# jianhengLiu/VINS-RGBD-FAST

Measured on AMD Instinct MI355X. Metric: VIO frames/sec (640x480, 150 feats, 10-KF window), higher is better.
Workload: dtype f64; 1 GPU; BASELINE configs[2]: 128 independent synthetic 640x480 RGB-D + 200 Hz IMU sequences per MI355X, 150 features, 10-keyframe window; sequences_per_gpu=128, tracker_lag=1, parallelism=sequences sharded per GPU, no data-path collective

## Files before the change

### vins-rgbd-fast_amd/csrc/be_linalg.h

```cpp
#pragma once
#include <hip/hip_runtime.h>
#include "vio_state.h"

namespace {

__device__ __forceinline__ double dpp_f64(double v, const int ctrl_tag) {
    int lo = __double2loint(v), hi = __double2hiint(v);
    switch (ctrl_tag) {
    case 0: lo = __builtin_amdgcn_update_dpp(0, lo, 0xB1, 0xF, 0xF, true); hi = __builtin_amdgcn_update_dpp(0, hi, 0xB1, 0xF, 0xF, true); break;
    case 1: lo = __builtin_amdgcn_update_dpp(0, lo, 0x4E, 0xF, 0xF, true); hi = __builtin_amdgcn_update_dpp(0, hi, 0x4E, 0xF, 0xF, true); break;
    case 2: lo = __builtin_amdgcn_update_dpp(0, lo, 0x141, 0xF, 0xF, true); hi = __builtin_amdgcn_update_dpp(0, hi, 0x141, 0xF, 0xF, true); break;
    default: lo = __builtin_amdgcn_update_dpp(0, lo, 0x140, 0xF, 0xF, true); hi = __builtin_amdgcn_update_dpp(0, hi, 0x140, 0xF, 0xF, true); break;
    }
    return __hiloint2double(hi, lo);
}
__device__ __forceinline__ double rl_f64(double v, int src_lane) {
    int lo = __double2loint(v), hi = __double2hiint(v);
    lo = __builtin_amdgcn_readlane(lo, src_lane);
    hi = __builtin_amdgcn_readlane(hi, src_lane);
    return __hiloint2double(hi, lo);
}
__device__ __forceinline__ double wave_sum_dpp(double v) {
    v += dpp_f64(v, 0);
    v += dpp_f64(v, 1);
// ... 1411 lines not shown
            WAVE_SYNC();
            if (lane < 16) xs[16 * p + lane] = x;
        }
        __syncthreads();
        for (int q = t; q < 16 * p; q += nt) {
            int tj = q >> 4, cc = q & 15;
            double sacc = 0;
#pragma unroll
            for (int k = 0; k < 16; k++) sacc += T[tl_idx(p, tj, k, cc)] * xs[16 * p + k];
            xs[q] -= sacc;
        }
        __syncthreads();
    }
}

__device__ __forceinline__ void chol_backward_tiles_wave(const double *T, int nb, double *xs, const double *dinv) {
    const int lane = threadIdx.x & 63, wave = threadIdx.x >> 6;
    if (wave == 0) {
        const int c = lane & 15;
        for (int p = nb - 1; p >= 0; p--) {
            const double *D = T + ((size_t)(p * (p + 1) / 2 + p) << 8);
            double m[16], b[16];
#pragma unroll
            for (int k = 0; k < 16; k++) { m[k] = D[(c << 4) + (k ^ c)]; b[k] = xs[16 * p + k]; }
            const double dv = dinv[16 * p + c];
            double x = 0;
#pragma unroll
            for (int k = 0; k < 16; k++) x += (k > c ? m[k] : (k == c ? dv : 0.0)) * b[k];
            WAVE_SYNC();
            if (lane < 16) xs[16 * p + lane] = x;
            WAVE_SYNC();
#pragma unroll
            for (int k = 0; k < 16; k++) b[k] = xs[16 * p + k];
            for (int q = lane; q < 16 * p; q += 64) {
                const int tj = q >> 4, cc = q & 15;
#pragma unroll
                for (int k = 0; k < 16; k++) m[k] = T[tl_idx(p, tj, k, cc)];
                double sacc = 0;
#pragma unroll
                for (int k = 0; k < 16; k++) sacc += m[k] * b[k];
                xs[q] -= sacc;
            }
            WAVE_SYNC();
        }
    }
    __syncthreads();
}

__device__ __forceinline__ void chol_solve_tiles(const double *T, int nb, double *xs, const double *dinv) {
    const int t = threadIdx.x, nt = blockDim.x, lane = t & 63, wave = t >> 6;
    for (int p = 0; p < nb; p++) {
        if (wave == 0) {
            const int row = lane & 15;
            double b = xs[16 * p + row];
#pragma unroll
            for (int j = 0; j < 16; j++) {
                double xj = bcast_lane(b, j) * dinv[16 * p + j];
                if (row == j) b = xj; else if (row > j) b -= T[tl_idx(p, p, row, j)] * xj;
            }
            if (lane < 16) xs[16 * p + row] = b;
// ... 293 lines not shown
        for (int a = t; a < n; a += nt) {
            double sacc = 0;
            if (a < n0 || (a >= e0 && a < e0 + ne))
                for (int q = 0; q < nw; q++) sacc += part[q * VIO_LWMAX + a];
            out_col[a] = sacc;
        }
    }
    __syncthreads();
}
template <int RB = 4>
__device__ __forceinline__ void matvec_pass_2range(const double *M, int ld, int nrows, int n, int n0, int e0, int ne, const double *u, const double *v,
                                                   double *out_col, double *out_row, double *part) {
    if (n0 + ne <= 128) matvec_pass_2range_t<2, RB>(M, ld, nrows, n, n0, e0, ne, u, v, out_col, out_row, part);
    else matvec_pass_t<6>(M, ld, nrows, n, u, v, out_col, out_row, part);
}
template <int RB = 4>
__device__ __forceinline__ void matvec_pass(const double *M, int ld, int nrows, int n, const double *u, const double *v, double *out_col, double *out_row,
                            double *part) {
    if (n <= 192) matvec_pass_t<3, RB>(M, ld, nrows, n, u, v, out_col, out_row, part);
    else matvec_pass_t<6>(M, ld, nrows, n, u, v, out_col, out_row, part);
}

}
```

### vins-rgbd-fast_amd/csrc/be_phased.h

```cpp
#define PS_LDS_TILE_DOUBLES 16896

namespace {

#define PS_LS_HEAD_DOUBLES (((int)(sizeof(Params) / sizeof(double)) + 1 & ~1) + 176)
#define PS_LVEC 14
__device__ __forceinline__ bool ps_active(const SolveSt &st) { return st.stage != PS_IDLE && st.stage != PS_DONE; }
__device__ __forceinline__ double *ps_imu_blk(const Ctx &c) { return c.pairblk + (size_t)((c.W + 1) * c.W / 2) * 210; }
__device__ __forceinline__ unsigned ps_colmask(int W1, int LW, bool vext) {
    unsigned m = 0;
    for (int cb = 0; cb < (LW >> 4); cb++) {
        const int c0 = 16 * cb, c1 = c0 + 15;
        if (c0 < 6 * W1 || (vext && c1 >= 15 * W1 && c0 < 15 * W1 + 7)) m |= 1u << cb;
    }
    return m;
}

__device__ __forceinline__ int fis_early(const SolveSt &st, int chunk, int pslot) { return st.fi[chunk][pslot]; }
__device__ __forceinline__ void ps_sel_rows(const Batch &B, Ctx &c, int buf) {
    if (!buf) return;
    const size_t S = (size_t)B.S, n8 = (size_t)c.NL + 8;
    c.Hpl += S * n8 * c.LW; c.Hll += S * n8; c.gl += S * n8;
}

}
// ... 143 lines not shown
            st.cost = ccost;
            st.succ++;
            if (rel < 0.25) st.radius *= 0.5;
            if (rel > 0.75) st.radius = fmax(st.radius, 3.0 * st.dogleg_norm);
            st.mu = fmax(1e-8, 2.0 * st.mu / 10.0);
            st.point_new = 1;
            if (st.fused && st.eval_with_J) st.rowbuf ^= 1;
            st.stage = st.iter >= cfg.max_iterations ? PS_DONE : PS_ASM;
        } else {
            st.radius *= 0.5;
            st.stage = st.iter >= cfg.max_iterations ? PS_DONE : PS_STEP;
        }
    }
}

__device__ __forceinline__ void ps_form_candidate(const Ctx &c, SolveSt &st, const double alpha, const double *delta, const double *stl, const double *sl, double *sred) {
    const int t = threadIdx.x, nt = blockDim.x;
    const vio_config &cfg = c.C->c;
    const int W = c.W, W1 = W + 1, oE = 15 * W1, oT = 15 * W1 + 6;
    const int F = st.F, Fa = st.Fa, ex_active = st.ex_active, td_active = st.td_active;
    const int *alist = c.pair_list + c.nres_cap - c.NL;
    const Params &X = st.X;
    Params &Xc = st.Xc;
    double xn2 = 0, dn2 = 0, ncl = 0;
    if (t <= W) {
        double pc[7], d6[6];
        for (int k = 0; k < 7; k++) pc[k] = X.pose[t * 7 + k];
        for (int k = 0; k < 6; k++) d6[k] = alpha * delta[6 * t + k];
        bf::pose_plus(pc, d6);
        for (int k = 0; k < 7; k++) { const double v = X.pose[t * 7 + k], d = v - pc[k]; xn2 += v * v; dn2 += d * d; Xc.pose[t * 7 + k] = pc[k]; }
        for (int k = 0; k < 9; k++) {
// ... 2 lines not shown
            Xc.sb[t * 9 + k] = vc;
        }
    }
    if (t == W + 1) {
        const bool relo = st.relo != 0;
        double ec[7], d6[6];
        for (int k = 0; k < 7; k++) ec[k] = relo ? X.relo[k] : X.ex[k];
        for (int k = 0; k < 6; k++) d6[k] = alpha * delta[oE + k];
        if (ex_active) bf::pose_plus(ec, d6);
        const double tdc = X.td + (td_active ? alpha * delta[oT] : 0.0);
        if (ex_active) for (int k = 0; k < 7; k++) { const double v = relo ? X.relo[k] : X.ex[k], d = v - ec[k]; xn2 += v * v; dn2 += d * d; }
        if (td_active) { xn2 += X.td * X.td; dn2 += (X.td - tdc) * (X.td - tdc); }
        for (int k = 0; k < 7; k++) { Xc.ex[k] = relo ? X.ex[k] : ec[k]; Xc.relo[k] = relo ? ec[k] : X.relo[k]; }
        Xc.td = tdc;
    }
    for (int k = t; k < F; k += nt) c.cfeat[k] = c.feat[k];
    __syncthreads();
    for (int k = t; k < Fa; k += nt) {
        int slot = alist[k], pi = c.lm_pidx[slot];
        const double v0 = c.feat[pi];
        double v = v0 + alpha * (stl[k] * sl[k]);
        double ub = (c.lm_est[slot] == 2) ? 2.0 / cfg.depth_max : 1.7976931348623157e308;
        if (v > ub) { v = ub; ncl += 1; }
        c.cfeat[pi] = v;
        xn2 += v0 * v0; dn2 += (v0 - v) * (v0 - v);
    }
    block_sum3(xn2, dn2, ncl, sred);
    if (t == 0) { st.step_xn2 = xn2; st.step_dn2 = dn2; if (ncl > 0) c.be->bound_clamps += (int)ncl; }
}

__device__ __forceinline__ bool ps_blk(const Batch &B, int &s, int &b) {
    if (B.xcd_nb == 0) { s = (int)blockIdx.y + B.s0; b = (int)blockIdx.x; return true; }
    const int L = (int)blockIdx.x, X = B.xcd_n, idx = L / X, sl = idx / B.xcd_nb, r = sl * X + (L - idx * X);
    b = idx - sl * B.xcd_nb;
    s = r + B.s0;
    return r < B.ns;
}
// ... 1292 lines not shown
    double *out = c.vec + 7 * LW;
    const int n0 = 6 * W1, e0 = 15 * W1, ne = st.vext ? 7 : 0;
    if (n0 + ne <= 128) ps_colsum_as_eight_waves<2, 8>(c.Hpl, LW, Fa, P, n0, e0, ne, wk_s, out, part);
    else ps_colsum_as_eight_waves<3, 8>(c.Hpl, LW, Fa, P, n0, e0, ne, wk_s, out, part);
}

__global__ __launch_bounds__(256, 5) void ps_asm_b_schur_kernel(Batch B, int nb_b, int by_blocks) {
    int s, b;
    if (!ps_blk(B, s, b)) return;
    extern __shared__ double ps_wk_s[];
    if (B.gn_ext && b == nb_b + B.n_schur) ps_gn_rhs_body(B, s, ps_wk_s);
    else if (b < nb_b) { if (by_blocks == 1) ps_asm_b_blocks(B, s, b, nb_b); else if (by_blocks == 2) ps_asm_b_body(B, s, b, nb_b, true); else ps_asm_b_body(B, s, b, nb_b, false); }
    else ps_schur_body(B, s, b - nb_b, ps_wk_s);
}

template <bool BIG, int TB> __device__ __forceinline__ void ps_serial_body(const Batch &B) {
    const int s = blockIdx.x + B.s0, t = threadIdx.x, nt = blockDim.x;
    SolveSt &st = B.sst[s];
    if (st.stage != PS_ASM && st.stage != PS_SCHUR && st.stage != PS_STEP) return;
    Ctx c = make_ctx(B, s);
    ps_sel_rows(B, c, st.rowbuf);
    const vio_config &cfg = c.C->c;
    const int W = c.W, W1 = W + 1, P = c.P, LW = c.LW;
    __shared__ double sred[64];
    __shared__ int sh_i[8];
    __shared__ double chol_dinv[VIO_LWMAX];
    extern __shared__ __attribute__((aligned(16))) unsigned char smem[];
    double *xs = (double *)smem, *work = xs + LW;
    const int F = st.F, Fa = st.Fa;
    const int ex_active = st.ex_active, td_active = st.td_active;
    const int ne_ext = st.vext ? 7 : 0;
// ... 7 lines not shown
           *yp = lv + 11 * LW, *up = lv + 12 * LW, *tmpv2 = lv + 13 * LW;
    double *sl = c.lvec, *dgl = c.lvec + c.NLs, *gradl = c.lvec + 2 * c.NLs, *gnl = c.lvec + 3 * c.NLs, *stl = c.lvec + 4 * c.NLs,
           *inv = c.lvec + 5 * c.NLs, *gls = c.lvec + 6 * c.NLs, *Hlls = c.lvec + 7 * c.NLs;
    const int Kpad = (Fa + 3) & ~3;
    double *hsgl = c.res + (size_t)c.nres_cap * 42 - 4 * (size_t)c.NLs;
    double *yl = hsgl + c.NLs, *ul = yl + c.NLs, *tmpl = ul + c.NLs;
    const int stage0 = st.stage;
    const bool s_formed = B.form_s && stage0 == PS_ASM && st.scale_pending == 0;
    double radius = st.radius, mu = st.mu, alpha = st.alpha, dogleg_norm = st.dogleg_norm;
    bool cauchy_valid = st.cauchy_valid != 0;
    int invalid = st.invalid;
    int iter = st.iter;
    if (!st.retry) iter++;
    PH_INIT;
    const bool have_lv = !(iter > cfg.max_iterations);
    if (have_lv) for (int i = t; i < PS_LVEC * LW; i += nt) lv[i] = c.vec[i];
    __syncthreads();
    auto finish = [&](int new_stage) {
        __syncthreads();
        if (have_lv) for (int i = 2 * LW + t; i < PS_LVEC * LW; i += nt) c.vec[i] = lv[i];
        if (t == 0) {
            st.radius = radius; st.mu = mu; st.alpha = alpha; st.dogleg_norm = dogleg_norm; st.cauchy_valid = cauchy_valid ? 1 : 0;
            st.invalid = invalid; st.iter = iter; st.stage = new_stage;
        }
    };
    if (iter > cfg.max_iterations) { if (t == 0) st.iters_done = cfg.max_iterations; iter = cfg.max_iterations; finish(PS_DONE); return; }
    if (t == 0) { st.iters_done = iter; st.retry = 0; }
    if (stage0 == PS_ASM || stage0 == PS_SCHUR) {
        if (st.scale_pending) {
            for (int k = t; k < Kpad; k += nt) sl[k] = k < Fa ? 1.0 / (1.0 + sqrt(c.Hll[k])) : 0.0;
            __syncthreads();
            if (t == 0) st.scale_pending = 0;
        }
        if (st.point_new) {
            double m = 0;
            for (int a = t; a < P; a += nt) m = fmax(m, sp[a] != 0.0 ? fabs(g[a]) : 0.0);
            for (int k = t; k < Fa; k += nt) m = fmax(m, fabs(c.gl[k]));
            const double gmax = block_max(m, sred);
            for (int a = t; a < LW; a += nt) {
                double hs = a < P ? sp[a] * sp[a] * c.H[a * LW + a] : 0.0;
                gs[a] = a < P ? sp[a] * g[a] : 0.0;
                dgp[a] = sqrt(fmin(fmax(hs, 1e-6), 1e32));
                gradp[a] = gs[a] / dgp[a];
                sgp[a] = gradp[a] / dgp[a];
                up[a] = sp[a] * sgp[a];
            }
            for (int k = t; k < Kpad; k += nt) {
                double hl = k < Fa ? sl[k] * sl[k] * c.Hll[k] : 0.0;
                Hlls[k] = hl;
                gls[k] = k < Fa ? sl[k] * c.gl[k] : 0.0;
                dgl[k] = sqrt(fmin(fmax(hl, 1e-6), 1e32));
                gradl[k] = gls[k] / dgl[k];
                ul[k] = sl[k] * (gradl[k] / dgl[k]);
            }
            __syncthreads();
            if (t == 0) st.point_new = 0;
            if (gmax <= 1e-10) { if (t == 0) st.iters_done = iter - 1; finish(PS_DONE); return; }
        }
        PH(48);
        cauchy_valid = false;
        for (int k = t; k < Kpad; k += nt) {
            double iv = k < Fa ? 1.0 / (Hlls[k] + mu * dgl[k] * dgl[k]) : 0.0;
            inv[k] = iv;
            if (!B.gn_ext) tmpl[k] = sl[k] * iv * gls[k];
        }
        __syncthreads();
        if (!B.gn_ext) matvec_pass_2range<TB>(c.Hpl, LW, Fa, P, 6 * W1, 15 * W1, ne_ext, tmpl, nullptr, tmpv, nullptr, work);
        for (int a = t; a < LW; a += nt) xs[a] = a < P ? gs[a] - sp[a] * tmpv[a] : 0.0;
        __syncthreads();
        PH(49);
        constexpr bool big = BIG;
        double *Stiles = big ? c.Sc : work;
        if (s_formed) {
            if (!big) {
                const int nd2 = (LW >> 4) * ((LW >> 4) + 1) / 2 * 128;
                const double2 *src = (const double2 *)c.Sc;
                double2 *dst = (double2 *)work;
                for (int i0 = t; i0 < nd2; i0 += 8 * nt) {
                    double2 v[8];
#pragma unroll
                    for (int u = 0; u < 8; u++) v[u] = src[min(i0 + u * nt, nd2 - 1)];
#pragma unroll
                    for (int u = 0; u < 8; u++) if (i0 + u * nt < nd2) dst[i0 + u * nt] = v[u];
                }
                __syncthreads();
            }
        } else {
            const unsigned colmask = ps_colmask(W1, LW, st.vext != 0);
            const int nb = LW >> 4, ntile = nb * (nb + 1) / 2;
// ... 18 lines not shown
                    sr[b] = sp[row]; sc0[b] = sp[col]; sc1[b] = sp[col + 1]; dg[b] = dgp[row];
                }
#pragma unroll
                for (int b = 0; b < TB; b++) {
                    if (tile0 + b * tstep >= ntile) break;
                    const double u0 = swp ? uv[b].y : uv[b].x, u1 = swp ? uv[b].x : uv[b].y;
                    double v0 = sr[b] * sc0[b] * (hv[b].x - u0), v1 = sr[b] * sc1[b] * (hv[b].y - u1);
                    if (dia0[b]) { v0 += mu * dg[b] * dg[b]; if (sr[b] == 0.0) v0 = 1.0; }
                    if (dia1[b]) { v1 += mu * dg[b] * dg[b]; if (sr[b] == 0.0) v1 = 1.0; }
                    *(double2 *)&Stiles[widx[b]] = swp ? make_double2(v1, v0) : make_double2(v0, v1);
                }
            }
            __syncthreads();
        }
        PH(50);
        bool ok = big ? chol_tiles_stream(c.Sc, LW >> 4, work, &sh_i[2], chol_dinv, xs)
                      : chol_tiles(work, LW >> 4, &sh_i[2], chol_dinv, s == 0 ? B.timings + 59 : nullptr, xs);
        PH(51);
        if (st.test_fail > 0) { ok = false; __syncthreads(); if (t == 0) st.test_fail--; }
        if (ok) {
            chol_backward_tiles_wave(big ? c.Sc : work, LW >> 4, xs, chol_dinv);
            PH(56);
            double bad = 0;
            for (int a = t; a < P; a += nt) if (!isfinite(xs[a])) bad += 1;
            bad = block_sum(bad, sred);
            ok = bad == 0;
        }
        if (!ok) {
            mu *= 10.0;
            if (mu < 1.0) { if (t == 0) st.retry = 1; finish(PS_SCHUR); return; }
            finish(PS_DONE);
            return;
        }
        PH(57);
        for (int a = t; a < LW; a += nt) { yp[a] = xs[a]; gnp[a] = -xs[a] * dgp[a]; tmpv[a] = sp[a] * xs[a]; }
        __syncthreads();
        matvec_pass_2range<TB>(c.Hpl, LW, Fa, P, 6 * W1, 15 * W1, ne_ext, nullptr, tmpv, nullptr, tmpl, nullptr);
        PH(58);
        for (int k = t; k < Kpad; k += nt) {
            double y = k < Fa ? (gls[k] - sl[k] * tmpl[k]) * inv[k] : 0.0;
            yl[k] = y;
            gnl[k] = -y * dgl[k];
        }
        __syncthreads();
    }
    PH(52);
    double gnorm = 0, gnn = 0, gdot = 0;
    for (int a = t; a < P; a += nt) { gnorm += gradp[a] * gradp[a]; gnn += gnp[a] * gnp[a]; gdot += gradp[a] * gnp[a]; }
    for (int k = t; k < Fa; k += nt) { gnorm += gradl[k] * gradl[k]; gnn += gnl[k] * gnl[k]; gdot += gradl[k] * gnl[k]; }
    block_sum3(gnorm, gnn, gdot, sred);
    gnorm = sqrt(gnorm);
    gnn = sqrt(gnn);
// ... 52 lines not shown
        }
    }
    block_sum3(n2, lin, quad, sred);
    if (dogleg_norm < 0) dogleg_norm = sqrt(n2);
    const double model_change = -(lin + 0.5 * quad);
    if (!(model_change > 0)) {
        if (++invalid >= 5) { finish(PS_DONE); return; }
        mu *= 10.0;
        finish(PS_SCHUR);
        return;
    }
    invalid = 0;
    PH(54);
    for (int a = t; a < LW; a += nt) delta[a] = a < P ? stp[a] * sp[a] : 0.0;
    __syncthreads();
    ps_form_candidate(c, st, 1.0, delta, stl, sl, sred);
    if (t == 0) st.ls_pending = st.constrained;
    if (t == 0) { st.model_change = model_change; st.eval_with_J = iter < cfg.max_iterations ? 1 : 0; }
    finish(PS_EVAL_C);
    PH(55);
}

__global__ __launch_bounds__(512) void ps_serial_kernel_512(Batch B) { ps_serial_body<false, 8>(B); }
__global__ __launch_bounds__(512) void ps_serial_big_kernel(Batch B) { ps_serial_body<true, 8>(B); }

__global__ __launch_bounds__(256, 2) void ps_ls_kernel(Batch B) {
    const int s = blockIdx.x + B.s0, t = threadIdx.x, nt = blockDim.x;
    SolveSt &st = B.sst[s];
    if (st.stage != PS_EVAL_C || !st.ls_pending) return;
    extern __shared__ __attribute__((aligned(16))) unsigned char lds[];
    __shared__ double sred[64];
    Ctx c = make_ctx(B, s);
    ps_sel_rows(B, c, st.rowbuf);
    const BeSeq &be = *c.be;
    const vio_config &cfg = c.C->c;
    const int W = c.W, W1 = W + 1, P = c.P, Fa = st.Fa, nblk = min(PS_MAX_EVAL_BLOCKS, 3 + (st.nres + 256 * B.eval_rpt - 1) / (256 * B.eval_rpt));
    constexpr int XD = ((int)(sizeof(Params) / sizeof(double)) + 1) & ~1;
    Params &X = *(Params *)lds;
    double *lsw = (double *)lds + XD, *lpart = lsw + 104;
// ... 90 lines not shown
```

### vins-rgbd-fast_amd/csrc/kernels.h

```cpp
#pragma once
#include <hip/hip_runtime.h>
#include "vio_state.h"
#include "../../include/vio_synth.h"

#define PI_CH 8
#define PREINT_MANY_LDS_DOUBLES (PI_CH * (225 + 270))
static inline size_t fast_lds_bytes(int rw, int rh) {
    return (size_t)(((rw + 6) * rh + 15) & ~15) + (size_t)((rw * rh + 15) & ~15) + (size_t)(((rw - 6) * (rh - 6) + 63) / 64 + 2) * 8 + 16;
}
__host__ __device__ static inline size_t ps_eval_lds_bytes(int W) {
    const size_t W1 = (size_t)W + 1, a = (W1 * W1 + 1) * 32 * 8, b = (size_t)W * (VIO_PREINT_HDR + 1) * 8;
    return (a > b ? a : b) + 64;
}
static inline size_t ps_ls_lds_bytes(int W) { (void)W; return ((((sizeof(Params) / sizeof(double)) + 1) & ~(size_t)1) + 176) * 8 + 16; }
struct LkImages {
    const uint8_t *prev[4];
    const uint8_t *next[4];
    int w[4], h[4];
};

__global__ void fe_begin_kernel(Batch B, const double *stamps, int gate, int publish, const uint8_t *modes, const double *R_rel);
__global__ void be_latest_odometry_kernel(Batch B, int seq, double *out11);
__global__ void fe_predict_motion_kernel(Batch B, int seq, double t0, double t1, double *out9);
__global__ void fe_pyrdown_kernel(Batch B, const uint8_t *src_base, size_t src_stride, int sw, int sh, int dst_level, int write_level0);
// ... 21 lines not shown
template <bool EXCALIB> __global__ void be_ingest_kernel(Batch B, const uint16_t *depth_base, size_t depth_stride, IngestSrc src);
__global__ void be_stage_relative_r_kernel(int n, const double *corres6, double *R9);
__global__ void be_solve_kernel(Batch B);
__global__ void be_solve_kernel_512(Batch B);
__global__ void be_marg_kernel(Batch B);
__global__ void be_marg_exact_kernel(Batch B);
__global__ void ps_setup_kernel(Batch B);
__global__ void ps_eval_kernel(Batch B);
__global__ void ps_eval_kernel_occ3(Batch B);
__global__ void ps_eval_kernel_occ4(Batch B);
__global__ void ps_asm_a_kernel(Batch B);
__global__ void ps_asm_a_kernel_occ4(Batch B);
__global__ void ps_asm_b_schur_kernel(Batch B, int nb_b, int by_blocks);
__global__ void ps_serial_big_kernel(Batch B);
__global__ void ps_serial_kernel_512(Batch B);
__global__ void ps_final_kernel(Batch B);
__global__ void ps_ls_kernel(Batch B);
__global__ void ps_evalf_kernel(Batch B);
static inline size_t ps_evalf_lds_bytes(int W) {
    const size_t W1 = (size_t)W + 1, a = ((size_t)PS_FUSE_CAP * 28 + (W1 * W / 2 + 1) * 32) * 8 + (size_t)PS_FUSE_CAP * 12, b = ((size_t)W * (VIO_PREINT_HDR + 1) + (size_t)W * 465) * 8;
    return (a > b ? a : b) + 16;
}
__global__ void be_prior_factor_kernel(Batch B, int seq);
__global__ void be_set_relo_kernel(Batch B, int seq, const double *par);
__global__ void be_stage_pnp_kernel(const double *pts, int n, double *par6);
__global__ void be_dyn_finalize_kernel(Batch B, int seq, const double *samples, const int *offs);
__global__ void be_stage_imu_kernel(vio_config cfg, PreInt *P, int n, const double *dt, const double *acc, const double *gyr,
                                    const double *par, double g_norm, double *preint_out, double *r15, double *J480);
__global__ void be_stage_projection_kernel(vio_config cfg, const double *in, int use_td, int form, double *r2, double *J46);
__global__ void be_stage_imu_block_kernel(const PreInt *P, const double *par, double g_norm, double *G961);
// ... 4 lines not shown
```

### vins-rgbd-fast_amd/csrc/vio_abi.hip

```cpp
#include <hip/hip_runtime.h>
#include <math.h>
#include <algorithm>
#include <cmath>
#include <stdlib.h>
#include <mutex>
#include <chrono>
#include <string>
#include <string.h>
#include <vector>
#include "kernels.h"
#include "dyninit_host.h"
#include "camera_model.h"
#include "snapshot.h"

thread_local std::string g_err;

namespace {

#define HIPCHK(x)                                                                                        \
    do {                                                                                                 \
        hipError_t e_ = (x);                                                                             \
        if (e_ != hipSuccess) { g_err = std::string(#x) + ": " + hipGetErrorString(e_); return VIO_EDEVICE; } \
    } while (0)

// ... 97 lines not shown
        bool busy = false;
    } imu_stage[2];
    int imu_stage_cur = 0;
    hipEvent_t ev_imu = nullptr;
    std::vector<double> last_imu_t;
    size_t lds_select = 0, lds_add = 0, lds_fast = 0, lds_solve = 0, lds_serial = 0, lds_marg = 0, lds_factor = 0, lds_ps_ls = 0, lds_ps_evalf = 0;
    int ps_evalf_blocks = 0;
    bool feed_throttle = true;
    int uploads_in_flight = 2;
    int relo_frames = 0;
    bool line_search = true;
    int be_threads = 512, marg_threads = 384;
    int solve_mode = 1;
    bool asm_a_occ4 = false;
    int eval_occ = 0;
    bool serial_big = false;
    size_t lds_ps_eval = 0;
    int ps_eval_blocks = 0, ps_asm_a_blocks = 0, ps_schur_tiles = 0;
    bool timing_valid = false;
    std::vector<hipEvent_t> pev;
    int prof_steps = 0, prof_cur = -1;
    bool prof_fe_only = false;
    struct SnapRow { const char *name; int kind; unsigned char *base; int64_t bytes, blob_off; };
    std::vector<SnapRow> snap_rows;
    int64_t snap_dev_bytes = 0, snap_chunks = 0;
    int snap_entries = 0;
    SnapEntry *d_snap_tab = nullptr;
    SnapSeq *d_snap_seqs = nullptr;
    size_t snap_seqs_cap = 0;
    unsigned char *d_snap_stage = nullptr;
// ... 516 lines not shown
            const dim3 g_e = xm ? dim3(S8 * nb_e) : dim3(nb_e, S), g_a = xm ? dim3(S8 * nb_a) : dim3(nb_a, S), g_b = xm ? dim3(S8 * nb_bs) : dim3(nb_bs, S);
            Batch Bf = Bg;
            Bf.ns = S; Bf.xcd_n = XN; Bf.xcd_nb = xm ? h->ps_evalf_blocks : 0;
            const dim3 g_f = xm ? dim3(S8 * h->ps_evalf_blocks) : dim3(h->ps_evalf_blocks, S);
            for (int k = 0; k < slots; k++) {
                if (Bg.fuse) ps_evalf_kernel<<<g_f, 256, h->lds_ps_evalf, st>>>(Bf);
                if (!fuse_only) {
                    if (h->eval_occ == 4) ps_eval_kernel_occ4<<<g_e, 256, h->lds_ps_eval, st>>>(Be);
                    else if (h->eval_occ == 3) ps_eval_kernel_occ3<<<g_e, 256, h->lds_ps_eval, st>>>(Be);
                    else ps_eval_kernel<<<g_e, 256, h->lds_ps_eval, st>>>(Be);
                    if (h->asm_a_occ4) ps_asm_a_kernel_occ4<<<g_a, 512, 0, st>>>(Ba);
                    else ps_asm_a_kernel<<<g_a, 512, 0, st>>>(Ba);
                }
                ps_asm_b_schur_kernel<<<g_b, 256, (size_t)(C.NL + 16 + (6 * (C.W + 1) + 7 <= 128 ? 8 * 128 : 8 * 192) ) * sizeof(double), st>>>(Bb, h->ps_asm_b_blocks, h->asm_b_by_blocks);
                if (h->serial_big) ps_serial_big_kernel<<<S, 512, h->lds_serial, st>>>(Bg);
                else ps_serial_kernel_512<<<S, 512, h->lds_serial, st>>>(Bg);
                if (h->line_search && k + 1 < slots) ps_ls_kernel<<<S, 256, h->lds_ps_ls, st>>>(Bg);
            }
            ps_final_kernel<<<S, 256, 0, st>>>(Bg);
        };
        if (h->use_graph && one_seq < 0) {
            uint64_t key = 1469598103934665603ULL;
            auto mixin = [&](const void *p, size_t nbytes) { const unsigned char *q = (const unsigned char *)p; for (size_t i = 0; i < nbytes; i++) { key ^= q[i]; key *= 1099511628211ULL; } };
            mixin(&Bg, sizeof(Bg));
            mixin(&h->line_search, sizeof(h->line_search));
            mixin(&fuse_only, sizeof(fuse_only));
            const int knobs[12] = {C.c.max_iterations + h->extra_slots, h->eval_occ, h->asm_a_occ4 ? 1 : 0, h->serial_big ? 1 : 0, h->serial_threads, h->ps_eval_blocks, h->ps_asm_a_blocks,
                                   h->ps_asm_b_blocks + 1000 * h->asm_b_by_blocks, h->ps_schur_tiles, h->xcd_map, h->xcd_n, (int)h->lds_serial};
            mixin(knobs, sizeof(knobs));
            mixin(&h->lds_ps_eval, sizeof(h->lds_ps_eval));
            if (g.solve_graph && g.solve_graph_key != key) { (void)hipGraphExecDestroy(g.solve_graph); g.solve_graph = nullptr; }
            g.solve_graph_key = key;
            if (!g.solve_graph) {
                hipGraph_t gr = nullptr;
                HIPCHK(hipStreamBeginCapture(st, hipStreamCaptureModeThreadLocal));
                launch_phased();
                HIPCHK(hipStreamEndCapture(st, &gr));
                HIPCHK(hipGraphInstantiate(&g.solve_graph, gr, nullptr, nullptr, 0));
                (void)hipGraphDestroy(gr);
            }
            HIPCHK(hipGraphLaunch(g.solve_graph, st));
        } else
// ... 316 lines not shown
            if (C.NPRIOR <= 96) workd = std::max(workd, (size_t)C.NPRIOR * (C.NPRIOR | 1) + 2);
            {
                size_t nb = (size_t)C.LW >> 4, tiles = nb * (nb + 1) / 2 * 256;
                if (tiles <= 16896) workd = std::max(workd, tiles);
            }
            h->lds_solve = ((size_t)C.LW + 2 + workd) * 8 + 16;
            (void)raise_lds_limit((const void *)be_solve_kernel, (size_t)(h->lds_solve));
            (void)raise_lds_limit((const void *)be_solve_kernel_512, (size_t)(h->lds_solve));
            {
                const size_t nb = (size_t)C.LW >> 4, tiles = nb * (nb + 1) / 2 * 256;
                const size_t wk = std::max(tiles <= 16896 ? tiles : (2 * nb + 1) * 256, (size_t)16 * 336);
                h->serial_big = tiles > 16896;
                h->B.form_s = (getenv("VIO_FORM_S") ? atoi(getenv("VIO_FORM_S")) != 0 : true) && h->asm_b_by_blocks == 2;
                h->lds_serial = ((size_t)C.LW + 2 + wk + 2 + (size_t)14  * C.LW) * 8 + 16;
                if (getenv("VIO_SERIAL_LDS") && (size_t)atol(getenv("VIO_SERIAL_LDS")) > h->lds_serial) h->lds_serial = (size_t)atol(getenv("VIO_SERIAL_LDS"));
                (void)raise_lds_limit(h->serial_big ? (const void *)ps_serial_big_kernel : (const void *)ps_serial_kernel_512, h->lds_serial);
            }
            {
                const size_t nb = (size_t)C.LW >> 4, tiles = nb * (nb + 1) / 2 * 256, W1 = (size_t)C.W + 1;
                const bool eligible = !(B.flags & 1) && (size_t)C.W * C.NP / 256 + 4 <= PS_MAX_EVAL_BLOCKS &&
                                      (size_t)C.W * 768 <= (W1 * W1 - W1 * C.W / 2) * 210 && nb <= 32;
                h->solve_mode = getenv("VIO_SOLVE_MODE") ? atoi(getenv("VIO_SOLVE_MODE")) : 1;
                if (!eligible) h->solve_mode = 0;
                h->lds_ps_eval = ps_eval_lds_bytes(C.W);
                (void)raise_lds_limit((const void *)ps_eval_kernel, h->lds_ps_eval);
                h->lds_ps_evalf = ps_evalf_lds_bytes(C.W);
                {
                    const int want = getenv("VIO_FUSE") ? atoi(getenv("VIO_FUSE")) : 0;
                    int chunks = (int)std::min<size_t>(PS_FUSE_MAXBLK, (W1 * (size_t)C.c.max_cnt * 11 / 10 + (PS_FUSE_CAP - C.W) - 1) / (PS_FUSE_CAP - C.W));
                    if (want > 1) chunks = std::min(PS_FUSE_MAXBLK, want);
                    B.fuse = (want && C.W <= PS_FUSE_MAXW && C.c.use_imu && B.pairpart) ? std::max(1, chunks) : 0;
// ... 29 lines not shown
        (void)raise_lds_limit((const void *)be_marg_kernel, (size_t)(h->lds_marg));
        (void)raise_lds_limit((const void *)be_marg_exact_kernel, (size_t)(h->lds_marg));
        const bool excalib = C.c.estimate_extrinsic == 2;
        const void *ingest = excalib ? (const void *)be_ingest_kernel<true> : (const void *)be_ingest_kernel<false>;
        (void)raise_lds_limit(ingest, ingest_lds_bytes(C, excalib));

        (void)raise_lds_limit((const void *)fe_select_kernel, (size_t)(h->lds_select));
        (void)raise_lds_limit((const void *)fe_add_kernel, (size_t)(h->lds_add));
        (void)raise_lds_limit((const void *)fe_fast_kernel, (size_t)(h->lds_fast));
        bool fits = lds_fits(C.MX > 0 ? (const void *)be_marg_exact_kernel : (const void *)be_marg_kernel, h->lds_marg, "be_marg") &&
                    lds_fits(ingest, ingest_lds_bytes(C, excalib), "be_ingest") &&
                    lds_fits((const void *)fe_select_kernel, h->lds_select, "fe_select") && lds_fits((const void *)fe_add_kernel, h->lds_add, "fe_add") &&
                    lds_fits((const void *)fe_fast_kernel, h->lds_fast, "fe_fast");
        if (fits && h->solve_mode == 1)
            fits = lds_fits((const void *)ps_eval_kernel, h->lds_ps_eval, "ps_eval") && lds_fits((const void *)ps_ls_kernel, h->lds_ps_ls, "ps_ls") &&
                   lds_fits(h->serial_big ? (const void *)ps_serial_big_kernel : (const void *)ps_serial_kernel_512, h->lds_serial, "ps_serial");
        else if (fits)
            fits = lds_fits(h->be_threads <= 512 ? (const void *)be_solve_kernel_512 : (const void *)be_solve_kernel, h->lds_solve, "be_solve");
        if (!fits) rc = VIO_ECAPACITY;
    }
    if (rc != VIO_OK) { vio_destroy(h); return nullptr; }
    return h;
}

void vio_destroy(vio_batch *h) {
    if (!h) return;
    int caller_dev = -1;
    const bool dev_switched = h->device >= 0 && hipGetDevice(&caller_dev) == hipSuccess && caller_dev != h->device && hipSetDevice(h->device) == hipSuccess;
    (void)hipDeviceSynchronize();
    for (void *p : h->allocs) (void)hipFree(p);
    if (h->d_gray_stage) (void)hipFree(h->d_gray_stage);
// ... 1658 lines not shown
```

Before: 60270 frames/s.

## Overlap serial-solve loads with compute via async LDS DMA and register prefetch

Adds an overlapped variant of the phased serial solver kernel, on by default and switchable with VIO_SERIAL_OVERLAP. At kernel start it issues global_load_lds DMA of the Schur tiles into LDS and prefetches per-thread scalars (Hll, gl, H diagonal, feature values, landmark indices) into registers so later stages skip those global reads. During the single-wave Cholesky back-substitution, the other waves prefetch Hpl rows into registers for the following row-dot pass. This hides global memory latency behind serial work, at the cost of higher register pressure in a 512-thread kernel and extra code complexity.

```diff
diff --git a/vins-rgbd-fast_amd/csrc/be_linalg.h b/vins-rgbd-fast_amd/csrc/be_linalg.h
--- a/vins-rgbd-fast_amd/csrc/be_linalg.h
+++ b/vins-rgbd-fast_amd/csrc/be_linalg.h
@@ -1449,9 +1449,9 @@
     }
 }
 
-__device__ __forceinline__ void chol_backward_tiles_wave(const double *T, int nb, double *xs, const double *dinv) {
-    const int lane = threadIdx.x & 63, wave = threadIdx.x >> 6;
-    if (wave == 0) {
+__device__ __forceinline__ void chol_backward_tiles_wave0(const double *T, int nb, double *xs, const double *dinv) {
+    const int lane = threadIdx.x & 63;
+    {
         const int c = lane & 15;
         for (int p = nb - 1; p >= 0; p--) {
             const double *D = T + ((size_t)(p * (p + 1) / 2 + p) << 8);
@@ -1479,6 +1479,9 @@
             WAVE_SYNC();
         }
     }
+}
+__device__ __forceinline__ void chol_backward_tiles_wave(const double *T, int nb, double *xs, const double *dinv) {
+    if ((threadIdx.x >> 6) == 0) chol_backward_tiles_wave0(T, nb, xs, dinv);
     __syncthreads();
 }
 
@@ -1802,6 +1805,64 @@
     if (n0 + ne <= 128) matvec_pass_2range_t<2, RB>(M, ld, nrows, n, n0, e0, ne, u, v, out_col, out_row, part);
     else matvec_pass_t<6>(M, ld, nrows, n, u, v, out_col, out_row, part);
 }
+template <int PR>
+__device__ __forceinline__ void rowdot_2range_prefetch(const double *M, int ld, int nrows, int n0, int e0, int ne, double (&m)[PR][2]) {
+    const int lane = threadIdx.x & 63, wave = threadIdx.x >> 6, nw = blockDim.x >> 6;
+    const int ncomp = n0 + ne;
+    int col[2];
+#pragma unroll
+    for (int j = 0; j < 2; j++) { const int q = lane + 64 * j; col[j] = q < n0 ? q : (q < ncomp ? e0 + (q - n0) : -1); }
+#pragma unroll
+    for (int b = 0; b < PR; b++) {
+        const double *r = M + (size_t)max(min((wave - 1) + (nw - 1) * b, nrows - 1), 0) * ld;
+#pragma unroll
+        for (int j = 0; j < 2; j++) m[b][j] = col[j] >= 0 ? r[col[j]] : 0.0;
+    }
+}
+template <int PR, int RB>
+__device__ __forceinline__ void rowdot_2range_finish(const double *M, int ld, int nrows, int n0, int e0, int ne, const double *v, double *out_row, const double (&m)[PR][2]) {
+    const int lane = threadIdx.x & 63, wave = threadIdx.x >> 6, nw = blockDim.x >> 6;
+    const int ncomp = n0 + ne;
+    int col[2];
+    double vv[2];
+#pragma unroll
+    for (int j = 0; j < 2; j++) {
+        const int q = lane + 64 * j;
+        col[j] = q < n0 ? q : (q < ncomp ? e0 + (q - n0) : -1);
+        vv[j] = col[j] >= 0 ? v[col[j]] : 0.0;
+    }
+    if (wave > 0) {
+#pragma unroll
+        for (int b = 0; b < PR; b++) {
+            const int k = (wave - 1) + (nw - 1) * b;
+            double rd = 0;
+#pragma unroll
+            for (int j = 0; j < 2; j++) rd += m[b][j] * vv[j];
+            rd = wave_sum_dpp(rd);
+            if (lane == 0 && k < nrows) out_row[k] = rd;
+        }
+    }
+    for (int k0 = (nw - 1) * PR + wave; k0 < nrows; k0 += RB * nw) {
+        double mr[RB][2];
+#pragma unroll
+        for (int b = 0; b < RB; b++) {
+            const double *r = M + (size_t)min(k0 + b * nw, nrows - 1) * ld;
+#pragma unroll
+            for (int j = 0; j < 2; j++) mr[b][j] = col[j] >= 0 ? r[col[j]] : 0.0;
+        }
+#pragma unroll
+        for (int b = 0; b < RB; b++) {
+            const int k = k0 + b * nw;
+            if (k >= nrows) break;
+            double rd = 0;
+#pragma unroll
+            for (int j = 0; j < 2; j++) rd += mr[b][j] * vv[j];
+            rd = wave_sum_dpp(rd);
+            if (lane == 0) out_row[k] = rd;
+        }
+    }
+    __syncthreads();
+}
 template <int RB = 4>
 __device__ __forceinline__ void matvec_pass(const double *M, int ld, int nrows, int n, const double *u, const double *v, double *out_col, double *out_row,
                             double *part) {
diff --git a/vins-rgbd-fast_amd/csrc/be_phased.h b/vins-rgbd-fast_amd/csrc/be_phased.h
--- a/vins-rgbd-fast_amd/csrc/be_phased.h
+++ b/vins-rgbd-fast_amd/csrc/be_phased.h
@@ -3,6 +3,7 @@
 namespace {
 
 #define PS_LS_HEAD_DOUBLES (((int)(sizeof(Params) / sizeof(double)) + 1 & ~1) + 176)
+#define PS_HPL_PRE 16
 #define PS_LVEC 14
 __device__ __forceinline__ bool ps_active(const SolveSt &st) { return st.stage != PS_IDLE && st.stage != PS_DONE; }
 __device__ __forceinline__ double *ps_imu_blk(const Ctx &c) { return c.pairblk + (size_t)((c.W + 1) * c.W / 2) * 210; }
@@ -181,7 +182,8 @@
     }
 }
 
-__device__ __forceinline__ void ps_form_candidate(const Ctx &c, SolveSt &st, const double alpha, const double *delta, const double *stl, const double *sl, double *sred) {
+struct CandPre { bool on; int slot, pi, est; double v0, sl0, f0; };
+__device__ __forceinline__ void ps_form_candidate(const Ctx &c, SolveSt &st, const double alpha, const double *delta, const double *stl, const double *sl, double *sred, const CandPre pre = CandPre{false, 0, 0, 0, 0.0, 0.0, 0.0}) {
     const int t = threadIdx.x, nt = blockDim.x;
     const vio_config &cfg = c.C->c;
     const int W = c.W, W1 = W + 1, oE = 15 * W1, oT = 15 * W1 + 6;
@@ -214,13 +216,14 @@
         for (int k = 0; k < 7; k++) { Xc.ex[k] = relo ? X.ex[k] : ec[k]; Xc.relo[k] = relo ? ec[k] : X.relo[k]; }
         Xc.td = tdc;
     }
-    for (int k = t; k < F; k += nt) c.cfeat[k] = c.feat[k];
+    for (int k = t; k < F; k += nt) c.cfeat[k] = (pre.on && k == t) ? pre.f0 : c.feat[k];
     __syncthreads();
     for (int k = t; k < Fa; k += nt) {
-        int slot = alist[k], pi = c.lm_pidx[slot];
-        const double v0 = c.feat[pi];
-        double v = v0 + alpha * (stl[k] * sl[k]);
-        double ub = (c.lm_est[slot] == 2) ? 2.0 / cfg.depth_max : 1.7976931348623157e308;
+        const bool f = pre.on && k == t;
+        int slot = f ? pre.slot : alist[k], pi = f ? pre.pi : c.lm_pidx[slot];
+        const double v0 = f ? pre.v0 : c.feat[pi];
+        double v = v0 + alpha * (stl[k] * (f ? pre.sl0 : sl[k]));
+        double ub = ((f ? pre.est : c.lm_est[slot]) == 2) ? 2.0 / cfg.depth_max : 1.7976931348623157e308;
         if (v > ub) { v = ub; ncl += 1; }
         c.cfeat[pi] = v;
         xn2 += v0 * v0; dn2 += (v0 - v) * (v0 - v);
@@ -1543,7 +1546,8 @@
     else ps_schur_body(B, s, b - nb_b, ps_wk_s);
 }
 
-template <bool BIG, int TB> __device__ __forceinline__ void ps_serial_body(const Batch &B) {
+template <bool BIG, int TB, bool OVL> __device__ __forceinline__ void ps_serial_body(const Batch &B) {
+    constexpr bool ovl = OVL && !BIG;
     const int s = blockIdx.x + B.s0, t = threadIdx.x, nt = blockDim.x;
     SolveSt &st = B.sst[s];
     if (st.stage != PS_ASM && st.stage != PS_SCHUR && st.stage != PS_STEP) return;
@@ -1581,6 +1585,28 @@
     if (!st.retry) iter++;
     PH_INIT;
     const bool have_lv = !(iter > cfg.max_iterations);
+    const bool dma_s = ovl && s_formed && B.gn_ext && have_lv;
+    const bool pre = ovl && have_lv && stage0 != PS_STEP;
+    const int scale_pending0 = st.scale_pending, point_new0 = st.point_new;
+    double r_hd = 0, r_gl = 0, r_hll = 0, r_sl = 0, r_hl = 0, r_gls = 0, r_dgl = 0;
+    CandPre cpre = {false, 0, 0, 0, 0.0, 0.0, 0.0};
+    if constexpr (ovl) {
+        if (dma_s) {
+            const int nd2 = nbk * (nbk + 1) / 2 * 128;
+            const double2 *src = (const double2 *)c.Sc + (t & 63);
+            for (int i0 = t & ~63; i0 < nd2; i0 += nt)
+                __builtin_amdgcn_global_load_lds((const __attribute__((address_space(1))) void *)(src + i0), (__attribute__((address_space(3))) void *)((double2 *)work + i0), 16, 0, 0);
+        }
+        if (pre) {
+            if (t < P) r_hd = c.H[t * LW + t];
+            if (t < Fa) { r_gl = c.gl[t]; r_hll = c.Hll[t]; cpre.slot = alist[t]; }
+            if (t < Kpad) {
+                if (!scale_pending0) r_sl = sl[t];
+                if (!point_new0) { r_hl = Hlls[t]; r_gls = gls[t]; r_dgl = dgl[t]; }
+            }
+            if (t < F) cpre.f0 = c.feat[t];
+        }
+    }
     if (have_lv) for (int i = t; i < PS_LVEC * LW; i += nt) lv[i] = c.vec[i];
     __syncthreads();
     auto finish = [&](int new_stage) {
@@ -1594,18 +1620,25 @@
     if (iter > cfg.max_iterations) { if (t == 0) st.iters_done = cfg.max_iterations; iter = cfg.max_iterations; finish(PS_DONE); return; }
     if (t == 0) { st.iters_done = iter; st.retry = 0; }
     if (stage0 == PS_ASM || stage0 == PS_SCHUR) {
-        if (st.scale_pending) {
-            for (int k = t; k < Kpad; k += nt) sl[k] = k < Fa ? 1.0 / (1.0 + sqrt(c.Hll[k])) : 0.0;
+        if (scale_pending0) {
+            for (int k = t; k < Kpad; k += nt) {
+                const double v = k < Fa ? 1.0 / (1.0 + sqrt(pre && k == t ? r_hll : c.Hll[k])) : 0.0;
+                sl[k] = v;
+                if (pre && k == t) r_sl = v;
+            }
             __syncthreads();
             if (t == 0) st.scale_pending = 0;
         }
-        if (st.point_new) {
+        if constexpr (ovl) {
+            if (pre && t < Fa) { cpre.pi = c.lm_pidx[cpre.slot]; cpre.est = c.lm_est[cpre.slot]; }
+        }
+        if (point_new0) {
             double m = 0;
             for (int a = t; a < P; a += nt) m = fmax(m, sp[a] != 0.0 ? fabs(g[a]) : 0.0);
-            for (int k = t; k < Fa; k += nt) m = fmax(m, fabs(c.gl[k]));
+            for (int k = t; k < Fa; k += nt) m = fmax(m, fabs(pre && k == t ? r_gl : c.gl[k]));
             const double gmax = block_max(m, sred);
             for (int a = t; a < LW; a += nt) {
-                double hs = a < P ? sp[a] * sp[a] * c.H[a * LW + a] : 0.0;
+                double hs = a < P ? sp[a] * sp[a] * (pre && a == t ? r_hd : c.H[a * LW + a]) : 0.0;
                 gs[a] = a < P ? sp[a] * g[a] : 0.0;
                 dgp[a] = sqrt(fmin(fmax(hs, 1e-6), 1e32));
                 gradp[a] = gs[a] / dgp[a];
@@ -1613,12 +1646,18 @@
                 up[a] = sp[a] * sgp[a];
             }
             for (int k = t; k < Kpad; k += nt) {
-                double hl = k < Fa ? sl[k] * sl[k] * c.Hll[k] : 0.0;
+                const bool f = pre && k == t;
+                const double slk = f ? r_sl : sl[k];
+                double hl = k < Fa ? slk * slk * (f ? r_hll : c.Hll[k]) : 0.0;
                 Hlls[k] = hl;
-                gls[k] = k < Fa ? sl[k] * c.gl[k] : 0.0;
-                dgl[k] = sqrt(fmin(fmax(hl, 1e-6), 1e32));
-                gradl[k] = gls[k] / dgl[k];
-                ul[k] = sl[k] * (gradl[k] / dgl[k]);
+                const double glsk = k < Fa ? slk * (f ? r_gl : c.gl[k]) : 0.0;
+                gls[k] = glsk;
+                const double dglk = sqrt(fmin(fmax(hl, 1e-6), 1e32));
+                dgl[k] = dglk;
+                const double gradlk = glsk / dglk;
+                gradl[k] = gradlk;
+                ul[k] = slk * (gradlk / dglk);
+                if (f) { r_hl = hl; r_gls = glsk; r_dgl = dglk; }
             }
             __syncthreads();
             if (t == 0) st.point_new = 0;
@@ -1627,9 +1666,14 @@
         PH(48);
         cauchy_valid = false;
         for (int k = t; k < Kpad; k += nt) {
-            double iv = k < Fa ? 1.0 / (Hlls[k] + mu * dgl[k] * dgl[k]) : 0.0;
+            const bool f = pre && k == t;
+            const double dglk = f ? r_dgl : dgl[k];
+            double iv = k < Fa ? 1.0 / ((f ? r_hl : Hlls[k]) + mu * dglk * dglk) : 0.0;
             inv[k] = iv;
-            if (!B.gn_ext) tmpl[k] = sl[k] * iv * gls[k];
+            if (!B.gn_ext) tmpl[k] = (f ? r_sl : sl[k]) * iv * (f ? r_gls : gls[k]);
+        }
+        if constexpr (ovl) {
+            if (pre && t < Fa) cpre.v0 = c.feat[cpre.pi];
         }
         __syncthreads();
         if (!B.gn_ext) matvec_pass_2range<TB>(c.Hpl, LW, Fa, P, 6 * W1, 15 * W1, ne_ext, tmpl, nullptr, tmpv, nullptr, work);
@@ -1639,7 +1683,7 @@
         constexpr bool big = BIG;
         double *Stiles = big ? c.Sc : work;
         if (s_formed) {
-            if (!big) {
+            if (!big && !dma_s) {
                 const int nd2 = (LW >> 4) * ((LW >> 4) + 1) / 2 * 128;
                 const double2 *src = (const double2 *)c.Sc;
                 double2 *dst = (double2 *)work;
@@ -1688,12 +1732,19 @@
             __syncthreads();
         }
         PH(50);
+        constexpr bool hpl_pre = ovl;
+        double hpl_m[ovl ? PS_HPL_PRE : 1][2];
         bool ok = big ? chol_tiles_stream(c.Sc, LW >> 4, work, &sh_i[2], chol_dinv, xs)
                       : chol_tiles(work, LW >> 4, &sh_i[2], chol_dinv, s == 0 ? B.timings + 59 : nullptr, xs);
         PH(51);
         if (st.test_fail > 0) { ok = false; __syncthreads(); if (t == 0) st.test_fail--; }
         if (ok) {
-            chol_backward_tiles_wave(big ? c.Sc : work, LW >> 4, xs, chol_dinv);
+            if constexpr (ovl) {
+                if (t < 64) chol_backward_tiles_wave0(work, LW >> 4, xs, chol_dinv);
+                else if constexpr (hpl_pre) rowdot_2range_prefetch<PS_HPL_PRE>(c.Hpl, LW, Fa, 6 * W1, 15 * W1, ne_ext, hpl_m);
+                __syncthreads();
+            } else
+                chol_backward_tiles_wave(big ? c.Sc : work, LW >> 4, xs, chol_dinv);
             PH(56);
             double bad = 0;
             for (int a = t; a < P; a += nt) if (!isfinite(xs[a])) bad += 1;
@@ -1709,7 +1760,11 @@
         PH(57);
         for (int a = t; a < LW; a += nt) { yp[a] = xs[a]; gnp[a] = -xs[a] * dgp[a]; tmpv[a] = sp[a] * xs[a]; }
         __syncthreads();
-        matvec_pass_2range<TB>(c.Hpl, LW, Fa, P, 6 * W1, 15 * W1, ne_ext, nullptr, tmpv, nullptr, tmpl, nullptr);
+        if constexpr (ovl) {
+            if constexpr (hpl_pre) rowdot_2range_finish<PS_HPL_PRE, TB>(c.Hpl, LW, Fa, 6 * W1, 15 * W1, ne_ext, tmpv, tmpl, hpl_m);
+            else matvec_pass_2range<TB>(c.Hpl, LW, Fa, P, 6 * W1, 15 * W1, ne_ext, nullptr, tmpv, nullptr, tmpl, nullptr);
+        } else
+            matvec_pass_2range<TB>(c.Hpl, LW, Fa, P, 6 * W1, 15 * W1, ne_ext, nullptr, tmpv, nullptr, tmpl, nullptr);
         PH(58);
         for (int k = t; k < Kpad; k += nt) {
             double y = k < Fa ? (gls[k] - sl[k] * tmpl[k]) * inv[k] : 0.0;
@@ -1792,15 +1847,17 @@
     PH(54);
     for (int a = t; a < LW; a += nt) delta[a] = a < P ? stp[a] * sp[a] : 0.0;
     __syncthreads();
-    ps_form_candidate(c, st, 1.0, delta, stl, sl, sred);
+    if constexpr (ovl) { if (pre) { cpre.on = true; cpre.sl0 = r_sl; } }
+    ps_form_candidate(c, st, 1.0, delta, stl, sl, sred, cpre);
     if (t == 0) st.ls_pending = st.constrained;
     if (t == 0) { st.model_change = model_change; st.eval_with_J = iter < cfg.max_iterations ? 1 : 0; }
     finish(PS_EVAL_C);
     PH(55);
 }
 
-__global__ __launch_bounds__(512) void ps_serial_kernel_512(Batch B) { ps_serial_body<false, 8>(B); }
-__global__ __launch_bounds__(512) void ps_serial_big_kernel(Batch B) { ps_serial_body<true, 8>(B); }
+__global__ __launch_bounds__(512) void ps_serial_kernel_512(Batch B) { ps_serial_body<false, 8, true>(B); }
+__global__ __launch_bounds__(512) void ps_serial_kernel_512_seq(Batch B) { ps_serial_body<false, 8, false>(B); }
+__global__ __launch_bounds__(512) void ps_serial_big_kernel(Batch B) { ps_serial_body<true, 8, false>(B); }
 
 __global__ __launch_bounds__(256, 2) void ps_ls_kernel(Batch B) {
     const int s = blockIdx.x + B.s0, t = threadIdx.x, nt = blockDim.x;
diff --git a/vins-rgbd-fast_amd/csrc/kernels.h b/vins-rgbd-fast_amd/csrc/kernels.h
--- a/vins-rgbd-fast_amd/csrc/kernels.h
+++ b/vins-rgbd-fast_amd/csrc/kernels.h
@@ -59,6 +59,7 @@
 __global__ void ps_asm_b_schur_kernel(Batch B, int nb_b, int by_blocks);
 __global__ void ps_serial_big_kernel(Batch B);
 __global__ void ps_serial_kernel_512(Batch B);
+__global__ void ps_serial_kernel_512_seq(Batch B);
 __global__ void ps_final_kernel(Batch B);
 __global__ void ps_ls_kernel(Batch B);
 __global__ void ps_evalf_kernel(Batch B);
diff --git a/vins-rgbd-fast_amd/csrc/vio_abi.hip b/vins-rgbd-fast_amd/csrc/vio_abi.hip
--- a/vins-rgbd-fast_amd/csrc/vio_abi.hip
+++ b/vins-rgbd-fast_amd/csrc/vio_abi.hip
@@ -135,6 +135,7 @@
     int solve_mode = 1;
     bool asm_a_occ4 = false;
     int eval_occ = 0;
+    bool serial_overlap = true;
     bool serial_big = false;
     size_t lds_ps_eval = 0;
     int ps_eval_blocks = 0, ps_asm_a_blocks = 0, ps_schur_tiles = 0;
@@ -681,7 +682,8 @@
                 }
                 ps_asm_b_schur_kernel<<<g_b, 256, (size_t)(C.NL + 16 + (6 * (C.W + 1) + 7 <= 128 ? 8 * 128 : 8 * 192) ) * sizeof(double), st>>>(Bb, h->ps_asm_b_blocks, h->asm_b_by_blocks);
                 if (h->serial_big) ps_serial_big_kernel<<<S, 512, h->lds_serial, st>>>(Bg);
-                else ps_serial_kernel_512<<<S, 512, h->lds_serial, st>>>(Bg);
+                else if (h->serial_overlap) ps_serial_kernel_512<<<S, 512, h->lds_serial, st>>>(Bg);
+                else ps_serial_kernel_512_seq<<<S, 512, h->lds_serial, st>>>(Bg);
                 if (h->line_search && k + 1 < slots) ps_ls_kernel<<<S, 256, h->lds_ps_ls, st>>>(Bg);
             }
             ps_final_kernel<<<S, 256, 0, st>>>(Bg);
@@ -692,7 +694,7 @@
             mixin(&Bg, sizeof(Bg));
             mixin(&h->line_search, sizeof(h->line_search));
             mixin(&fuse_only, sizeof(fuse_only));
-            const int knobs[12] = {C.c.max_iterations + h->extra_slots, h->eval_occ, h->asm_a_occ4 ? 1 : 0, h->serial_big ? 1 : 0, h->serial_threads, h->ps_eval_blocks, h->ps_asm_a_blocks,
+            const int knobs[13] = {h->serial_overlap ? 1 : 0, C.c.max_iterations + h->extra_slots, h->eval_occ, h->asm_a_occ4 ? 1 : 0, h->serial_big ? 1 : 0, h->serial_threads, h->ps_eval_blocks, h->ps_asm_a_blocks,
                                    h->ps_asm_b_blocks + 1000 * h->asm_b_by_blocks, h->ps_schur_tiles, h->xcd_map, h->xcd_n, (int)h->lds_serial};
             mixin(knobs, sizeof(knobs));
             mixin(&h->lds_ps_eval, sizeof(h->lds_ps_eval));
@@ -1039,7 +1041,8 @@
                 h->B.form_s = (getenv("VIO_FORM_S") ? atoi(getenv("VIO_FORM_S")) != 0 : true) && h->asm_b_by_blocks == 2;
                 h->lds_serial = ((size_t)C.LW + 2 + wk + 2 + (size_t)14  * C.LW) * 8 + 16;
                 if (getenv("VIO_SERIAL_LDS") && (size_t)atol(getenv("VIO_SERIAL_LDS")) > h->lds_serial) h->lds_serial = (size_t)atol(getenv("VIO_SERIAL_LDS"));
-                (void)raise_lds_limit(h->serial_big ? (const void *)ps_serial_big_kernel : (const void *)ps_serial_kernel_512, h->lds_serial);
+                h->serial_overlap = getenv("VIO_SERIAL_OVERLAP") ? atoi(getenv("VIO_SERIAL_OVERLAP")) != 0 : true;
+                (void)raise_lds_limit((h->serial_big ? (const void *)ps_serial_big_kernel : h->serial_overlap ? (const void *)ps_serial_kernel_512 : (const void *)ps_serial_kernel_512_seq), h->lds_serial);
             }
             {
                 const size_t nb = (size_t)C.LW >> 4, tiles = nb * (nb + 1) / 2 * 256, W1 = (size_t)C.W + 1;
@@ -1099,7 +1102,7 @@
                     lds_fits((const void *)fe_fast_kernel, h->lds_fast, "fe_fast");
         if (fits && h->solve_mode == 1)
             fits = lds_fits((const void *)ps_eval_kernel, h->lds_ps_eval, "ps_eval") && lds_fits((const void *)ps_ls_kernel, h->lds_ps_ls, "ps_ls") &&
-                   lds_fits(h->serial_big ? (const void *)ps_serial_big_kernel : (const void *)ps_serial_kernel_512, h->lds_serial, "ps_serial");
+                   lds_fits((h->serial_big ? (const void *)ps_serial_big_kernel : h->serial_overlap ? (const void *)ps_serial_kernel_512 : (const void *)ps_serial_kernel_512_seq), h->lds_serial, "ps_serial");
         else if (fits)
             fits = lds_fits(h->be_threads <= 512 ? (const void *)be_solve_kernel_512 : (const void *)be_solve_kernel, h->lds_solve, "be_solve");
         if (!fits) rc = VIO_ECAPACITY;
```

Result: no change. 60580 frames/s (median of 6 runs) (+0.5%).
